# nianticlabs/mickey

Hardware: NVIDIA H100
Metric: image-pairs/sec @720x540 (higher is better)
Workload: dtype f16 operands / f32 accumulate (tensor core), f32 matcher+solver

## Files before the change

### mickey_b200/csrc/epilogue.cuh

```cuda
#pragma once
#include "common.cuh"

namespace mk {

__device__ __forceinline__ float rcp_approx(float x) { float y; asm("rcp.approx.ftz.f32 %0, %1;" : "=f"(y) : "f"(x)); return y; }
__device__ __forceinline__ float ex2_approx_f(float x) { float y; asm("ex2.approx.ftz.f32 %0, %1;" : "=f"(y) : "f"(x)); return y; }
__device__ __forceinline__ float gelu_erf(float x) {
  const float z = fabsf(x) * 0.70710678118654752f;
  const float t = rcp_approx(fmaf(0.3275911f, z, 1.0f));
  float poly = fmaf(1.061405429f, t, -1.453152027f);
  poly = fmaf(poly, t, 1.421413741f);
  poly = fmaf(poly, t, -0.284496736f);
  poly = fmaf(poly, t, 0.254829592f);
  const float erf_abs = fmaf(-poly * t, ex2_approx_f(-1.4426950408889634f * z * z), 1.0f);
  const float hx = 0.5f * x;
  return fmaf(hx, copysignf(erf_abs, x), hx);
}

__device__ __forceinline__ void fma2_f32(float& d0, float& d1, float a0, float a1, float b0, float b1, float c0, float c1) {
  d0 = __fmaf_rn(a0, b0, c0);
  d1 = __fmaf_rn(a1, b1, c1);
}
__device__ __forceinline__ void mul2_f32(float& d0, float& d1, float a0, float a1, float b0, float b1) {
  d0 = __fmul_rn(a0, b0);
// ... 105 lines not shown
        uint4 u = r[q];
        const __half2* h = reinterpret_cast<const __half2*>(&u);
#pragma unroll
        for (int e = 0; e < 4; ++e) {
          float2 f = __half22float2(h[e]);
          v[q * 8 + e * 2] += f.x;
          v[q * 8 + e * 2 + 1] += f.y;
        }
      }
    }
#pragma unroll
    for (int j = 0; j < 32; ++j) v[j] = apply_act(v[j], p.act);
    if (p.aux && ((p.aux_group_mask >> g) & 1)) add_vec32(v, p.aux + (size_t)pos * p.N + n0);
    if (!valid) {
#pragma unroll
      for (int j = 0; j < 32; ++j) v[j] = 0.0f;
    }
    if (p.out_f) {
      float* o = p.out_f + (size_t)g * p.out_f_group_off + (size_t)m * p.out_f_ld + n0;
#pragma unroll
      for (int q = 0; q < 8; ++q)
        reinterpret_cast<float4*>(o)[q] = make_float4(v[q * 4], v[q * 4 + 1], v[q * 4 + 2], v[q * 4 + 3]);
    }
    if (p.out_h) store_h32(p.out_h + (size_t)g * p.out_h_group_off + (size_t)m * p.out_h_ld + n0, v);
  } else if constexpr (EPI == EPI_STORE_F) {
    if (m >= p.M) return;
    float* o = p.out_f + (size_t)g * p.out_f_group_off + (size_t)m * p.out_f_ld + n0;
#pragma unroll
    for (int q = 0; q < 8; ++q)
      reinterpret_cast<float4*>(o)[q] = make_float4(v[q * 4], v[q * 4 + 1], v[q * 4 + 2], v[q * 4 + 3]);
  }
}

template <int CPL> struct VecF;
template <> struct VecF<1> { using T = float; };
template <> struct VecF<2> { using T = float2; };

template <int CPL> __device__ __forceinline__ void ld_f(const float* p, float (&v)[CPL]) {
  if constexpr (CPL == 2) { const float2 t = *reinterpret_cast<const float2*>(p); v[0] = t.x; v[1] = t.y; } else { v[0] = *p; }
}
template <int CPL> __device__ __forceinline__ void ldg_f(const float* p, float (&v)[CPL]) {
  if constexpr (CPL == 2) { const float2 t = __ldg(reinterpret_cast<const float2*>(p)); v[0] = t.x; v[1] = t.y; } else { v[0] = __ldg(p); }
}
template <int CPL> __device__ __forceinline__ void st_f(float* p, const float (&v)[CPL]) {
  if constexpr (CPL == 2) { *reinterpret_cast<float2*>(p) = make_float2(v[0], v[1]); } else { *p = v[0]; }
}
template <int CPL> __device__ __forceinline__ void st_h(__half* p, const float (&v)[CPL]) {
  if constexpr (CPL == 2) { *reinterpret_cast<__half2*>(p) = __floats2half2_rn(v[0], v[1]); } else { *p = __float2half_rn(v[0]); }
}
template <int CPL> __device__ __forceinline__ void ld_h(const __half* p, float (&v)[CPL]) {
  if constexpr (CPL == 2) { const float2 t = __half22float2(*reinterpret_cast<const __half2*>(p)); v[0] = t.x; v[1] = t.y; }
  else { v[0] = __half2float(*p); }
}

__device__ __forceinline__ float warp_rowsum32(float (&part)[32], int lane) {
#pragma unroll
  for (int o = 16; o >= 1; o >>= 1) {
    const bool upper = (lane & o) != 0;
#pragma unroll
    for (int i = 0; i < o; ++i) {
      const float send = upper ? part[i] : part[i + o];
      const float keep = upper ? part[i + o] : part[i];
      part[i] = keep + __shfl_xor_sync(0xffffffffu, send, o);
    }
  }
  return part[0];
}

__device__ __forceinline__ float resid_ln_pass1(const GemmParams& p, int row0, int lane, int col_base, float* stage) {
  constexpr int LDS = 64 + 4, RB = 8;
  const int col = col_base + lane * 2;
  const float2 bias = __ldg(reinterpret_cast<const float2*>(p.bias + col)), gam = __ldg(reinterpret_cast<const float2*>(p.gamma + col));
  const int rows = min(32, p.M - row0);
  float part[32];
#pragma unroll
  for (int r0 = 0; r0 < 32; r0 += RB) {
    float2 v[RB], x[RB];
#pragma unroll
    for (int i = 0; i < RB; ++i) {
      const int r = r0 + i;
      v[i] = *reinterpret_cast<const float2*>(stage + r * LDS + lane * 2);
      x[i] = make_float2(0.f, 0.f);
      if (r < rows) x[i] = *reinterpret_cast<const float2*>(p.out_f + (size_t)(row0 + r) * p.out_f_ld + col);
    }
#pragma unroll
    for (int i = 0; i < RB; ++i) {
      const int r = r0 + i;
      float2 y = make_float2(0.f, 0.f);
      if (r < rows) {
        y.x = fmaf(gam.x, v[i].x + bias.x, x[i].x); y.y = fmaf(gam.y, v[i].y + bias.y, x[i].y);
        *reinterpret_cast<float2*>(p.out_f + (size_t)(row0 + r) * p.out_f_ld + col) = y;
      }
      *reinterpret_cast<float2*>(stage + r * LDS + lane * 2) = y;
      part[r] = y.x + y.y;
    }
  }
  return warp_rowsum32(part, lane);
}

__device__ __forceinline__ float resid_ln_pass2(int lane, const float* stage, float mean_l) {
  constexpr int LDS = 64 + 4;
  float part[32];
#pragma unroll
  for (int r = 0; r < 32; ++r) {
    const float2 x = *reinterpret_cast<const float2*>(stage + r * LDS + lane * 2);
    const float mean = __shfl_sync(0xffffffffu, mean_l, r);
    const float d0 = x.x - mean, d1 = x.y - mean;
    part[r] = d0 * d0 + d1 * d1;
  }
  return warp_rowsum32(part, lane);
}

__device__ __forceinline__ void resid_ln_pass3(const GemmParams& p, int row0, int lane, int col_base, const float* stage,
                                               float mean_l, float rstd_l) {
  constexpr int LDS = 64 + 4;
  const int col = col_base + lane * 2;
  const float2 w = __ldg(reinterpret_cast<const float2*>(p.aux + col)), b = __ldg(reinterpret_cast<const float2*>(p.beta + col));
  const int rows = min(32, p.M - row0);
#pragma unroll 8
  for (int r = 0; r < 32; ++r) {
    const float2 x = *reinterpret_cast<const float2*>(stage + r * LDS + lane * 2);
    const float mean = __shfl_sync(0xffffffffu, mean_l, r), rstd = __shfl_sync(0xffffffffu, rstd_l, r);
    if (r < rows)
      *reinterpret_cast<__half2*>(p.out_h + (size_t)(row0 + r) * p.out_h_ld + col) =
          __floats2half2_rn((x.x - mean) * rstd * w.x + b.x, (x.y - mean) * rstd * w.y + b.y);
  }
}

__device__ __forceinline__ void ld8(const float* p, float (&v)[8]) {
  const float4 a = *reinterpret_cast<const float4*>(p), b = *reinterpret_cast<const float4*>(p + 4);
  v[0] = a.x; v[1] = a.y; v[2] = a.z; v[3] = a.w; v[4] = b.x; v[5] = b.y; v[6] = b.z; v[7] = b.w;
}
__device__ __forceinline__ void ldg8(const float* p, float (&v)[8]) {
  const float4 a = __ldg(reinterpret_cast<const float4*>(p)), b = __ldg(reinterpret_cast<const float4*>(p) + 1);
  v[0] = a.x; v[1] = a.y; v[2] = a.z; v[3] = a.w; v[4] = b.x; v[5] = b.y; v[6] = b.z; v[7] = b.w;
}
__device__ __forceinline__ void st8(float* p, const float (&v)[8]) {
  reinterpret_cast<float4*>(p)[0] = make_float4(v[0], v[1], v[2], v[3]);
  reinterpret_cast<float4*>(p)[1] = make_float4(v[4], v[5], v[6], v[7]);
}
__device__ __forceinline__ void st8h(__half* p, const float (&v)[8]) {
  __half2 h0 = __floats2half2_rn(v[0], v[1]), h1 = __floats2half2_rn(v[2], v[3]);
  __half2 h2 = __floats2half2_rn(v[4], v[5]), h3 = __floats2half2_rn(v[6], v[7]);
  uint4 u;
  u.x = *reinterpret_cast<uint32_t*>(&h0); u.y = *reinterpret_cast<uint32_t*>(&h1);
  u.z = *reinterpret_cast<uint32_t*>(&h2); u.w = *reinterpret_cast<uint32_t*>(&h3);
  *reinterpret_cast<uint4*>(p) = u;
}
__device__ __forceinline__ void ld8h(const __half* p, float (&v)[8]) {
  const uint4 u = *reinterpret_cast<const uint4*>(p);
  const __half2* h = reinterpret_cast<const __half2*>(&u);
#pragma unroll
  for (int e = 0; e < 4; ++e) { const float2 f = __half22float2(h[e]); v[2 * e] = f.x; v[2 * e + 1] = f.y; }
}

template <int EPI, int W, int ACT>
__device__ __forceinline__ void epilogue_rows_impl(const GemmParams& p, int g, int row0, int lane, int col_base,
                                                   const float* __restrict__ stage, float mean_l, float rstd_l) {
  constexpr int LDS = W + 4;
  constexpr int LPR = W / 8;
  constexpr int RPS = 32 / LPR;
  constexpr int STEPS = 32 / RPS;
  constexpr bool GLOBAL_IN = (EPI == EPI_RESID_F || EPI == EPI_PATCH || EPI == EPI_CONV || EPI == EPI_LN);
  constexpr int U = GLOBAL_IN ? 2 : 4;
  static_assert(W % 8 == 0 && 32 % LPR == 0 && STEPS % U == 0, "staged epilogue: W in {32, 64}");
  const int seg = lane % LPR, rsub = lane / LPR;
  const int col = col_base + seg * 8;
  float bias[8], gam[8], bet[8];
#pragma unroll
  for (int i = 0; i < 8; ++i) { bias[i] = 0.f; gam[i] = 1.f; bet[i] = 0.f; }
  if constexpr (EPI == EPI_STORE_H || EPI == EPI_CONV) { if (p.bias) ldg8(p.bias + (size_t)g * p.bias_group_off + col, bias); }
  if constexpr (EPI == EPI_RESID_F) { ldg8(p.bias + col, bias); ldg8(p.gamma + col, gam); }
  if constexpr (EPI == EPI_LN) { ldg8(p.gamma + (size_t)g * p.ln_group_off + col, gam); ldg8(p.beta + (size_t)g * p.ln_group_off + col, bet); }
  const bool use_aux = (EPI == EPI_CONV) && p.aux && ((p.aux_group_mask >> g) & 1);
  const bool use_res = (EPI == EPI_CONV) && p.res_h;
  const bool ln_res = (EPI == EPI_LN) && p.out_f;
  const int rows = min(32, p.M - row0);
  int my_pos = 0, my_valid = 1, my_orow = 0;
  {
    const int mr = row0 + lane;
    if constexpr (EPI == EPI_CONV || EPI == EPI_LN) {
      if (p.pad_h2) { int pos; my_valid = pad_valid(p, mr, pos) ? 1 : 0; my_pos = pos; }
    }
    if constexpr (EPI == EPI_PATCH) {
      const int img = mr / p.tok_per_img;
      my_pos = mr - img * p.tok_per_img;
      my_orow = img * (p.tok_per_img + 1) + 1 + my_pos;
    }
  }
  float* out_f = p.out_f ? p.out_f + (size_t)g * p.out_f_group_off + col : nullptr;
  __half* out_h = p.out_h ? p.out_h + (size_t)g * p.out_h_group_off + col : nullptr;
#pragma unroll 1
  for (int s0 = 0; s0 < STEPS; s0 += U) {
    float v[U][8], x[U][8], a[U][8];
    int pos[U], orow[U];
    bool valid[U], live[U];
    float mean[U], rstd[U];
#pragma unroll
    for (int u = 0; u < U; ++u) {
      const int r = (s0 + u) * RPS + rsub;
      const size_t m = (size_t)(row0 + r);
      live[u] = r < rows;
      ld8(stage + r * LDS + seg * 8, v[u]);
      pos[u] = __shfl_sync(0xffffffffu, my_pos, r);
      orow[u] = __shfl_sync(0xffffffffu, my_orow, r);
      valid[u] = __shfl_sync(0xffffffffu, my_valid, r) != 0;
      mean[u] = 0.f; rstd[u] = 0.f;
      if constexpr (EPI == EPI_LN) { mean[u] = __shfl_sync(0xffffffffu, mean_l, r); rstd[u] = __shfl_sync(0xffffffffu, rstd_l, r); }
#pragma unroll
      for (int k = 0; k < 8; ++k) { x[u][k] = 0.f; a[u][k] = 0.f; }
      if (live[u]) {
        if constexpr (EPI == EPI_RESID_F) ld8(out_f + m * p.out_f_ld, x[u]);
        if constexpr (EPI == EPI_PATCH) ldg8(p.aux + (size_t)pos[u] * p.N + col, a[u]);
        if constexpr (EPI == EPI_CONV) {
          if (use_res) ld8h(p.res_h + (size_t)g * p.res_h_group_off + m * p.res_h_ld + col, x[u]);
          if (use_aux) ldg8(p.aux + (size_t)pos[u] * p.N + col, a[u]);
        }
        if constexpr (EPI == EPI_LN) { if (ln_res) ld8(out_f + m * p.out_f_ld, x[u]); }
      }
    }
#pragma unroll
    for (int u = 0; u < U; ++u) {
      if (!live[u]) continue;
      const int r = (s0 + u) * RPS + rsub;
      const size_t m = (size_t)(row0 + r);
      if constexpr (EPI == EPI_STORE_H) {
        if constexpr (ACT == ACT_GELU) {
#pragma unroll
          for (int k = 0; k < 8; k += 2) gelu_erf2(v[u][k] + bias[k], v[u][k + 1] + bias[k + 1], v[u][k], v[u][k + 1]);
        } else {
#pragma unroll
          for (int k = 0; k < 8; ++k) {
            const float t = v[u][k] + bias[k];
            v[u][k] = (ACT == ACT_RELU) ? fmaxf(t, 0.f) : t;
          }
        }
// ... 216 lines not shown
```

### mickey_b200/csrc/gemm.cu

```cuda
#include "gemm.h"
#include "gemm_tc.cuh"

#include <algorithm>
#include <cstdarg>
#include <cstdlib>
#include <cstring>
#include <mutex>
#include <unordered_map>

namespace mk {

typedef CUresult (*PFN_encodeTiled)(CUtensorMap*, CUtensorMapDataType, cuuint32_t, void*, const cuuint64_t*,
                                    const cuuint64_t*, const cuuint32_t*, const cuuint32_t*, CUtensorMapInterleave,
                                    CUtensorMapSwizzle, CUtensorMapL2promotion, CUtensorMapFloatOOBfill);

static PFN_encodeTiled get_encode() {
  static PFN_encodeTiled fn = nullptr;
  static std::once_flag once;
  std::call_once(once, [] {
    void* p = nullptr;
    cudaDriverEntryPointQueryResult qres;
    if (cudaGetDriverEntryPoint("cuTensorMapEncodeTiled", &p, cudaEnableDefault, &qres) == cudaSuccess &&
        qres == cudaDriverEntryPointSuccess)
      fn = reinterpret_cast<PFN_encodeTiled>(p);
// ... 161 lines not shown
    for (int c = 0; c < BN / 32; ++c) {
      if (n0 + c * 32 < p.N) {
        for (int j = 0; j < 32; ++j) v[j] = acc[c * 32 + j];
        epilogue_chunk<EPI>(p, g, m, n0 + c * 32, v);
      }
    }
  }
}

bool pdl_enabled() {
  static int v = -1;
  if (v < 0) { const char* e = getenv("MICKEY_PDL"); v = (e && strcmp(e, "0") == 0) ? 0 : 1; }
  return v == 1;
}

static bool use_simt() {
  static int v = -1;
  if (v < 0) {
    const char* e = getenv("MICKEY_GEMM_IMPL");
    v = (e && strcmp(e, "simt") == 0) ? 1 : 0;
  }
  return v == 1;
}

int sm_count() {
  static int n[64] = {0};
  int dev = 0;
  cudaGetDevice(&dev);
  int& c = n[dev & 63];
  if (!c) { cudaDeviceGetAttribute(&c, cudaDevAttrMultiProcessorCount, dev); if (c <= 0) c = 132; }
  return c;
}

template <int BN, int EPI, int STAGES, bool PERSISTENT>
static int launch_tc(const CUtensorMap& tmA, const CUtensorMap& tmB, const GemmParams& p, cudaStream_t stream,
                     const OutMaps& om = no_out_maps()) {
  static unsigned long long attr_mask = 0;
  constexpr int smem = gemm_smem_bytes<BN, EPI, STAGES, PERSISTENT>();
  if (first_use_on_device(attr_mask)) {
    MK_CUDA_CHECK(cudaFuncSetAttribute(gemm_tc_kernel<BN, EPI, STAGES, PERSISTENT>, cudaFuncAttributeMaxDynamicSharedMemorySize, smem));
  }
  const int tiles = gemm_tile_count<BN>(p);
  cudaLaunchConfig_t cfg = {};
  cfg.gridDim = dim3(PERSISTENT ? std::min(tiles, sm_count()) : tiles);
  cfg.blockDim = dim3(gemm_threads<PERSISTENT>()); cfg.dynamicSmemBytes = smem; cfg.stream = stream;
  cudaLaunchAttribute attr[2];
  int n_attr = 0;
  if (pdl_enabled()) {
    attr[n_attr].id = cudaLaunchAttributeProgrammaticStreamSerialization;
    attr[n_attr++].val.programmaticStreamSerializationAllowed = 1;
  }
  if constexpr (EPI == EPI_RESID_LN) {
    attr[n_attr].id = cudaLaunchAttributeClusterDimension;
    attr[n_attr].val.clusterDim.x = p.N / BN; attr[n_attr].val.clusterDim.y = 1; attr[n_attr++].val.clusterDim.z = 1;
  }
  cfg.attrs = attr;
  cfg.numAttrs = n_attr;
  MK_CUDA_CHECK(cudaLaunchKernelEx(&cfg, gemm_tc_kernel<BN, EPI, STAGES, PERSISTENT>, tmA, tmB, p, om));
  return MK_OK;
}

static bool deep_ring(int tiles, const GemmParams& p) {
  return (long long)tiles <= (long long)sm_count() * 5 / 4 && p.k_chunks > 3;
}
static bool persistent_grid(int tiles) { return tiles > 8 * sm_count(); }

template <int BN, int EPI>
static int launch_one(const GemmOperand& A, const GemmOperand& B, const GemmParams& p, cudaStream_t stream, int impl) {
  const int tiles = gemm_tile_count<BN>(p);
  if constexpr (EPI == EPI_RESID_LN) {
    if (impl == GEMM_IMPL_SIMT || BN != 128 || p.N / BN > 8 || p.groups != 1) { set_last_error("EPI_RESID_LN: wgmma path, N <= 1024, one group"); return MK_ERR_UNSUPPORTED; }
  }
  if (impl == GEMM_IMPL_SIMT) {
    if constexpr (EPI != EPI_RESID_LN)
    MK_CUDA_CHECK(launch_k(gemm_simt_kernel<BN, EPI>, dim3(tiles), dim3(128), 0, stream, reinterpret_cast<const __half*>(A.ptr),
                           (long long)A.rows, (long long)A.ld, reinterpret_cast<const __half*>(B.ptr), (long long)B.rows,
                           (long long)B.ld, p));
  } else {
    CUtensorMap tmA, tmB;
    int rc = make_tensor_map_f16(&tmA, A.ptr, A.rows, A.cols, A.ld, BLOCK_M);
    if (rc) return rc;
    rc = make_tensor_map_f16(&tmB, B.ptr, B.rows, B.cols, B.ld, BN);
    if (rc) return rc;
    if constexpr (EPI == EPI_DUAL) {
      if (p.out_tma) {
        OutMaps om = {};
        float* outs[3] = {p.scores, p.kp_scores, p.final_scores};
        for (int i = 0; i < 3; ++i)
          if (outs[i]) { rc = encode_tensor_map_out_f32(&om.m[i], outs[i], p.n_valid, p.out_pitch, p.groups); if (rc) return rc; }
        return launch_tc<BN, EPI, shallow_stages<BN>(), false>(tmA, tmB, p, stream, om);
      }
    }
    if (deep_ring(tiles, p)) return launch_tc<BN, EPI, deep_stages<BN>(), false>(tmA, tmB, p, stream);
    if constexpr (persistent_epilogue<EPI>())
      if (persistent_grid(tiles)) return launch_tc<BN, EPI, ring_stages<BN>(), true>(tmA, tmB, p, stream);
    return launch_tc<BN, EPI, shallow_stages<BN>(), false>(tmA, tmB, p, stream);
  }
  MK_CUDA_CHECK(cudaGetLastError());
  return MK_OK;
}

template <int EPI>
static int launch_bn(int bn, const GemmOperand& A, const GemmOperand& B, const GemmParams& p, cudaStream_t s, int impl) {
  if (bn == 128) return launch_one<128, EPI>(A, B, p, s, impl);
  if (bn == 64) return launch_one<64, EPI>(A, B, p, s, impl);
  set_last_error("unsupported BLOCK_N %d", bn);
  return MK_ERR_INVALID;
}

bool gemm_resid_ln_supported(int M, int N, int k_chunks) {
  (void)M; (void)k_chunks;
  static int on = -1;
  if (on < 0) { const char* e = getenv("MICKEY_FUSE_LN"); on = (e && e[0] == '1') ? 1 : 0; }
  return on && !use_simt() && N % 128 == 0 && N <= 1024;
}

int launch_gemm(int epi, const GemmOperand& A, const GemmOperand& B, const GemmParams& p, cudaStream_t stream, int impl) {
  if (impl == GEMM_IMPL_DEFAULT) impl = use_simt() ? GEMM_IMPL_SIMT : GEMM_IMPL_TC;
  if (p.k_chunks <= 0 || p.M <= 0 || p.N <= 0 || p.groups <= 0) { set_last_error("bad GEMM shape"); return MK_ERR_INVALID; }
  const bool matcher = (epi == EPI_LSE || epi == EPI_DUAL);
  if (matcher && impl == GEMM_IMPL_SIMT) { set_last_error("the matcher epilogues run on the wgmma kernel only"); return MK_ERR_UNSUPPORTED; }
  if (matcher && (p.part_ld % 128 || p.part_ld < p.n_valid)) { set_last_error("matcher: part_ld must be n_valid rounded up to 128"); return MK_ERR_INVALID; }
  if (epi == EPI_DUAL && p.out_pitch < p.n_valid) { set_last_error("matcher: out_pitch %lld < n_valid %d", p.out_pitch, p.n_valid); return MK_ERR_INVALID; }
  if (!matcher && (p.N % 32)) { set_last_error("GEMM N=%d must be a multiple of 32", p.N); return MK_ERR_INVALID; }
  int bn = (matcher || p.N % 128 == 0) ? 128 : 64;
  if (!matcher && p.N % bn) { set_last_error("GEMM N=%d not tileable", p.N); return MK_ERR_INVALID; }
  if (epi == EPI_LN && p.N != 128) { set_last_error("EPI_LN needs N == 128"); return MK_ERR_INVALID; }
  if (epi == EPI_RESID_LN && (p.N % 128 || p.N > 1024 || p.groups != 1 || !p.aux || !p.beta || !p.out_h || !p.out_f)) {
// ... 29 lines not shown
```

### mickey_b200/csrc/gemm.h

```cpp
#pragma once
#include "common.cuh"

namespace mk {

struct GemmOperand {
  const void* ptr;
  long long rows, cols, ld;
};

enum GemmImpl : int { GEMM_IMPL_DEFAULT = 0, GEMM_IMPL_TC = 1, GEMM_IMPL_SIMT = 2 };

int make_tensor_map_f16(CUtensorMap* map, const void* ptr, long long rows, long long cols, long long ld_elems, int box_rows);
int encode_tensor_map_2d(CUtensorMap* map, CUtensorMapDataType dtype, const void* ptr, long long rows, long long cols,
                         long long ld_elems, int box_rows);
int make_tensor_map_out_f16(CUtensorMap* map, void* ptr, long long groups, long long rows, long long cols, int box_rows);
int sm_count();
int launch_gemm(int epi, const GemmOperand& A, const GemmOperand& B, const GemmParams& p, cudaStream_t stream,
                int impl = GEMM_IMPL_DEFAULT);
bool gemm_resid_ln_supported(int M, int N, int k_chunks);
const char* last_error();

}
```

### mickey_b200/csrc/gemm_tc.cuh

```cuda
#pragma once
#include "common.cuh"
#include "epilogue.cuh"

namespace mk {

constexpr int BLOCK_M = 128;
constexpr int BLOCK_K = 64;
constexpr int WGMMA_K = 16;
constexpr int GEMM_WARP_EPI = 8;

template <int BN> constexpr int ring_stages() { return BN == 128 ? 4 : 6; }
template <int BN> constexpr int shallow_stages() { return BN == 128 ? 3 : 4; }
template <int BN> constexpr int deep_stages() { return BN == 128 ? 6 : 8; }
template <int EPI> constexpr bool persistent_epilogue() { return EPI != EPI_DUAL && EPI != EPI_RESID_LN && EPI != EPI_LN; }
template <bool PERSISTENT> constexpr int gemm_threads() { return PERSISTENT ? 640 : 288; }
template <bool PERSISTENT> constexpr int gemm_warp_tma() { return PERSISTENT ? 16 : 8; }

constexpr int DUAL_STAGE_BYTES = 3 * 4096;
constexpr int DUAL_AUX_BYTES = 8 * 64 * 4;
constexpr int DUAL_BYTES = 8 * DUAL_STAGE_BYTES + DUAL_AUX_BYTES;

template <int BN> constexpr int acc_block_floats() { return 32 * (BN / 2 + 4); }
template <int BN> constexpr int acc_tile_bytes() { return 8 * acc_block_floats<BN>() * 4; }
template <int BN, int STAGES> constexpr int ring_bytes() { return STAGES * (BLOCK_M * BLOCK_K * 2 + BN * BLOCK_K * 2); }
template <int BN, int EPI, int STAGES, bool PERSISTENT> constexpr int acc_tile_offset() {
  return PERSISTENT ? ring_bytes<BN, STAGES>() : EPI == EPI_DUAL ? DUAL_BYTES : 0;
}
template <int BN, int EPI, int STAGES, bool PERSISTENT>
constexpr int region_bytes() {
  return ring_bytes<BN, STAGES>() > acc_tile_offset<BN, EPI, STAGES, PERSISTENT>() + acc_tile_bytes<BN>()
             ? ring_bytes<BN, STAGES>() : acc_tile_offset<BN, EPI, STAGES, PERSISTENT>() + acc_tile_bytes<BN>();
}
template <int BN, int EPI, int STAGES, bool PERSISTENT> constexpr int gemm_smem_bytes() {
  return region_bytes<BN, EPI, STAGES, PERSISTENT>() + 1024 + 256 + 2048;
}
template <int BN, int EPI, int STAGES, bool PERSISTENT> constexpr int gemm_ctas_per_sm() {
  return !PERSISTENT && EPI != EPI_LN && EPI != EPI_RESID_LN && gemm_smem_bytes<BN, EPI, STAGES, PERSISTENT>() <= 113 * 1024 ? 2 : 1;
}

struct GemmTile { int g, m0, n0, n_tile; };
template <int BN>
__host__ __device__ __forceinline__ int gemm_tile_count(const GemmParams& p) {
  return ((p.M + BLOCK_M - 1) / BLOCK_M) * ((p.N + BN - 1) / BN) * p.groups;
}
template <int BN>
__device__ __forceinline__ GemmTile gemm_tile(const GemmParams& p, int t) {
  const int n_tiles = (p.N + BN - 1) / BN, m_tiles = (p.M + BLOCK_M - 1) / BLOCK_M;
  const int n = t % n_tiles;
  t /= n_tiles;
  int g, m;
  if (p.a_row_group_off == 0 && p.a_col_group_off == 0) { g = t % p.groups; m = t / p.groups; }
  else { m = t % m_tiles; g = t / m_tiles; }
  return {g, m * BLOCK_M, n * BN, n};
}

__device__ __forceinline__ uint32_t smem_u32(const void* p) { return (uint32_t)__cvta_generic_to_shared(p); }

__device__ __forceinline__ void mbar_init(uint32_t bar, uint32_t count) {
  asm volatile("mbarrier.init.shared::cta.b64 [%0], %1;" ::"r"(bar), "r"(count));
}
__device__ __forceinline__ void mbar_expect_tx(uint32_t bar, uint32_t bytes) {
  asm volatile("mbarrier.arrive.expect_tx.shared::cta.b64 _, [%0], %1;" ::"r"(bar), "r"(bytes) : "memory");
}
__device__ __forceinline__ void mbar_arrive(uint32_t bar) {
  asm volatile("mbarrier.arrive.shared::cta.b64 _, [%0];" ::"r"(bar) : "memory");
}
__device__ __forceinline__ void mbar_wait(uint32_t bar, uint32_t parity) {
  asm volatile(
      "{\n\t"
      ".reg .pred P1;\n\t"
      "WAIT_%=:\n\t"
      "mbarrier.try_wait.parity.shared::cta.b64 P1, [%0], %1;\n\t"
      "@P1 bra DONE_%=;\n\t"
      "bra WAIT_%=;\n\t"
      "DONE_%=:\n\t"
      "}" ::"r"(bar), "r"(parity) : "memory");
}
__device__ __forceinline__ void tma_load_2d(uint32_t dst, const CUtensorMap* map, uint32_t bar, int c0, int c1) {
  asm volatile(
      "cp.async.bulk.tensor.2d.shared::cluster.global.mbarrier::complete_tx::bytes [%0], [%1, {%3, %4}], [%2];"
      ::"r"(dst), "l"(map), "r"(bar), "r"(c0), "r"(c1) : "memory");
}
__device__ __forceinline__ bool elect_one() {
  uint32_t pred = 0;
  asm volatile(
      "{\n\t"
      ".reg .pred P1;\n\t"
      "elect.sync _|P1, 0xFFFFFFFF;\n\t"
      "selp.b32 %0, 1, 0, P1;\n\t"
      "}" : "=r"(pred));
  return pred != 0;
}
constexpr int GEMM_REGS_PRODUCER = 40;
constexpr int GEMM_REGS_EPILOGUE = 120;
template <int R> __device__ __forceinline__ void setmaxnreg_dec() { asm volatile("setmaxnreg.dec.sync.aligned.u32 %0;" ::"n"(R)); }
template <int R> __device__ __forceinline__ void setmaxnreg_inc() { asm volatile("setmaxnreg.inc.sync.aligned.u32 %0;" ::"n"(R)); }
__device__ __forceinline__ void consumer_sync() { asm volatile("bar.sync 1, 256;" ::: "memory"); }

__device__ __forceinline__ uint64_t gmma_desc_sw128(uint32_t smem_addr) {
  uint64_t d = 0;
  d |= (uint64_t)((smem_addr & 0x3FFFF) >> 4);
  d |= (uint64_t)1 << 16;
  d |= (uint64_t)(1024 >> 4) << 32;
  d |= (uint64_t)1 << 62;
  return d;
}
__device__ __forceinline__ void wgmma_fence() { asm volatile("wgmma.fence.sync.aligned;" ::: "memory"); }
__device__ __forceinline__ void wgmma_commit() { asm volatile("wgmma.commit_group.sync.aligned;" ::: "memory"); }
template <int N> __device__ __forceinline__ void wgmma_wait() { asm volatile("wgmma.wait_group.sync.aligned %0;" ::"n"(N) : "memory"); }
template <int N> __device__ __forceinline__ void reg_fence(float (&d)[N]) {
#pragma unroll
  for (int i = 0; i < N; ++i) asm volatile("" : "+f"(d[i])::"memory");
}

__device__ __forceinline__ void wgmma_m64n64k16(float (&d)[32], uint64_t desc_a, uint64_t desc_b, uint32_t scale_d) {
// ... 9 lines not shown
  asm volatile(
      "{\n\t.reg .pred p;\n\tsetp.ne.b32 p, %66, 0;\n\t"
      "wgmma.mma_async.sync.aligned.m64n128k16.f32.f16.f16 "
      "{%0, %1, %2, %3, %4, %5, %6, %7, %8, %9, %10, %11, %12, %13, %14, %15, %16, %17, %18, %19, %20, %21, %22, %23, %24, %25, %26, %27, %28, %29, %30, %31, %32, %33, %34, %35, %36, %37, %38, %39, %40, %41, %42, %43, %44, %45, %46, %47, %48, %49, %50, %51, %52, %53, %54, %55, %56, %57, %58, %59, %60, %61, %62, %63}, %64, %65, p, 1, 1, 0, 0;\n\t}"
      : "+f"(d[0]), "+f"(d[1]), "+f"(d[2]), "+f"(d[3]), "+f"(d[4]), "+f"(d[5]), "+f"(d[6]), "+f"(d[7]), "+f"(d[8]), "+f"(d[9]), "+f"(d[10]), "+f"(d[11]), "+f"(d[12]), "+f"(d[13]), "+f"(d[14]), "+f"(d[15]), "+f"(d[16]), "+f"(d[17]), "+f"(d[18]), "+f"(d[19]), "+f"(d[20]), "+f"(d[21]), "+f"(d[22]), "+f"(d[23]), "+f"(d[24]), "+f"(d[25]), "+f"(d[26]), "+f"(d[27]), "+f"(d[28]), "+f"(d[29]), "+f"(d[30]), "+f"(d[31]), "+f"(d[32]), "+f"(d[33]), "+f"(d[34]), "+f"(d[35]), "+f"(d[36]), "+f"(d[37]), "+f"(d[38]), "+f"(d[39]), "+f"(d[40]), "+f"(d[41]), "+f"(d[42]), "+f"(d[43]), "+f"(d[44]), "+f"(d[45]), "+f"(d[46]), "+f"(d[47]), "+f"(d[48]), "+f"(d[49]), "+f"(d[50]), "+f"(d[51]), "+f"(d[52]), "+f"(d[53]), "+f"(d[54]), "+f"(d[55]), "+f"(d[56]), "+f"(d[57]), "+f"(d[58]), "+f"(d[59]), "+f"(d[60]), "+f"(d[61]), "+f"(d[62]), "+f"(d[63])
      : "l"(desc_a), "l"(desc_b), "r"(scale_d));
}

template <int BN>
__device__ __forceinline__ void wgmma_tile(float (&d)[BN / 2], uint64_t desc_a, uint64_t desc_b, uint32_t scale_d) {
  if constexpr (BN == 128) wgmma_m64n128k16(d, desc_a, desc_b, scale_d);
  else wgmma_m64n64k16(d, desc_a, desc_b, scale_d);
}

__device__ __forceinline__ void cluster_sync_all() {
  asm volatile("barrier.cluster.arrive.release.aligned;\n\tbarrier.cluster.wait.acquire.aligned;" ::: "memory");
}
__device__ __forceinline__ uint32_t cluster_size() {
  uint32_t r;
  asm volatile("mov.u32 %0, %%cluster_nctarank;" : "=r"(r));
  return r;
}
__device__ __forceinline__ float ld_dsmem_f32(uint32_t local_smem_addr, uint32_t cta_rank) {
  uint32_t remote;
  asm volatile("mapa.shared::cluster.u32 %0, %1, %2;" : "=r"(remote) : "r"(local_smem_addr), "r"(cta_rank));
  float v;
  asm volatile("ld.shared::cluster.f32 %0, [%1];" : "=f"(v) : "r"(remote) : "memory");
  return v;
}

template <int BN>
__device__ __forceinline__ void acc_chunk(const float* acc, int q, int lane, int c, float (&v)[32]) {
  constexpr int W = BN / 2;
  const float4* src = reinterpret_cast<const float4*>(acc + (q + 4 * ((c * 32) / W)) * acc_block_floats<BN>() + lane * (W + 4) + (c * 32) % W);
#pragma unroll
  for (int k4 = 0; k4 < 8; ++k4) {
    const float4 t = src[k4];
    v[k4 * 4] = t.x; v[k4 * 4 + 1] = t.y; v[k4 * 4 + 2] = t.z; v[k4 * 4 + 3] = t.w;
  }
}

template <int BN, int EPI>
__device__ __forceinline__ void tile_epilogue(const GemmParams& p, const OutMaps& om, int g, int m0, int n0, int n_tile, int q, int half,
                                              int lane, float* acc, float* red, uint32_t red_saddr, float* dual_stage, float* dual_aux) {
  constexpr int CHUNKS = BN / 32;
  constexpr int W = BN / 2;
  constexpr int CPH = CHUNKS / 2;
  const int c_begin = half * CPH, c_end = c_begin + CPH;
  const int m = m0 + q * 32 + lane;
  float* stage = acc + (q + 4 * half) * acc_block_floats<BN>();
  float v[32];
  if constexpr (EPI == EPI_LN) {
    float sum = 0.f;
#pragma unroll
    for (int c = 0; c < CHUNKS; ++c) {
      acc_chunk<BN>(acc, q, lane, c, v);
#pragma unroll
      for (int j = 0; j < 32; ++j) sum += v[j];
    }
    const float mean = sum * (1.0f / BN);
    float sq = 0.f;
#pragma unroll
    for (int c = 0; c < CHUNKS; ++c) {
      acc_chunk<BN>(acc, q, lane, c, v);
#pragma unroll
      for (int j = 0; j < 32; ++j) { const float d = v[j] - mean; sq += d * d; }
    }
    const float rstd = rsqrtf(sq * (1.0f / BN) + p.eps);
    epilogue_rows<EPI_LN, W>(p, g, m0 + q * 32, lane, n0 + half * W, stage, mean, rstd);
  } else if constexpr (EPI == EPI_RESID_LN) {
// ... 41 lines not shown
    const bool row_ok = m < p.n_valid;
    const float lr = row_ok ? __ldg(p.lse_r + (size_t)g * p.part_ld + m) : -MK_NEG_INF;
    const float s0 = row_ok ? __ldg(p.scr0 + (size_t)g * p.n_valid + m) : 0.0f;
    if (p.out_tma) {
      float lc_pre[CPH], s1_pre[CPH];
#pragma unroll
      for (int ci = 0; ci < CPH; ++ci) {
        const int col = n0 + (c_begin + ci) * 32 + lane;
        const bool ok = col < p.n_valid;
        lc_pre[ci] = ok ? __ldg(p.lse_c + (size_t)g * p.part_ld + col) : -MK_NEG_INF;
        s1_pre[ci] = ok ? __ldg(p.scr1 + (size_t)g * p.n_valid + col) : 0.0f;
      }
#pragma unroll
      for (int ci = 0; ci < CPH; ++ci) {
        const int c = c_begin + ci;
        if (n0 + c * 32 < p.n_valid && m0 + q * 32 < p.n_valid) {
          acc_chunk<BN>(acc, q, lane, c, v);
          dual_store_chunk_tma(p, om, g, m0 + q * 32, lane, n0 + c * 32, v, dual_stage, dual_aux, lr, s0, lc_pre[ci], s1_pre[ci]);
        }
      }
    } else {
      for (int c = c_begin; c < c_end; ++c) {
        if (n0 + c * 32 < p.n_valid) {
          acc_chunk<BN>(acc, q, lane, c, v);
          dual_store_chunk(p, g, m0 + q * 32, lane, n0 + c * 32, v, dual_stage, lr, s0);
        }
      }
    }
  } else {
    epilogue_rows<EPI, W>(p, g, m0 + q * 32, lane, n0 + half * W, stage, 0.f, 0.f);
  }
}

template <int BN, int EPI, int STAGES, bool PERSISTENT>
__global__ void __launch_bounds__((gemm_threads<PERSISTENT>()), (gemm_ctas_per_sm<BN, EPI, STAGES, PERSISTENT>()))
gemm_tc_kernel(const __grid_constant__ CUtensorMap tmA, const __grid_constant__ CUtensorMap tmB, const GemmParams p,
               const __grid_constant__ OutMaps om) {
  static_assert(BN == 64 || BN == 128, "wgmma tiles: N = 64 or 128");
  static_assert(gemm_smem_bytes<BN, EPI, STAGES, PERSISTENT>() <= 227 * 1024, "GEMM: shared memory");
  extern __shared__ uint8_t smem_raw[];
  constexpr int A_BYTES = BLOCK_M * BLOCK_K * 2;
  constexpr int B_BYTES = BN * BLOCK_K * 2;
  constexpr int STAGE_BYTES = A_BYTES + B_BYTES;
  constexpr int W = BN / 2;
  static_assert(!PERSISTENT || persistent_epilogue<EPI>(), "this epilogue runs one tile per CTA");
  constexpr bool ONE_TILE = !PERSISTENT;
  constexpr int WARP_TMA = gemm_warp_tma<PERSISTENT>();

  const uint32_t raw = smem_u32(smem_raw);
  const uint32_t base = (raw + 1023u) & ~1023u;
  const uint32_t bar_base = base + region_bytes<BN, EPI, STAGES, PERSISTENT>();
  const uint32_t full_bar0 = bar_base;
  const uint32_t empty_bar0 = bar_base + 8 * STAGES;
  const uint32_t acc_full_bar = bar_base + 16 * STAGES;
  const uint32_t acc_empty_bar = acc_full_bar + 8;
  const uint32_t red_saddr = bar_base + 256;
  uint8_t* const gbase = smem_raw + (base - raw);
  float* const acc = reinterpret_cast<float*>(gbase + acc_tile_offset<BN, EPI, STAGES, PERSISTENT>());

  const int warp = threadIdx.x >> 5;
  const int lane = threadIdx.x & 31;
  const int n_tiles_total = gemm_tile_count<BN>(p);

  if (warp == WARP_TMA && lane == 0) {
    asm volatile("prefetch.tensormap [%0];" ::"l"(&tmA) : "memory");
    asm volatile("prefetch.tensormap [%0];" ::"l"(&tmB) : "memory");
    for (int s = 0; s < STAGES; ++s) {
      mbar_init(full_bar0 + 8 * s, 1);
      mbar_init(empty_bar0 + 8 * s, 8);
    }
    mbar_init(acc_full_bar, 256);
    mbar_init(acc_empty_bar, 256);
    asm volatile("fence.mbarrier_init.release.cluster;" ::: "memory");
  }
  __syncthreads();
  pdl_wait();

  if (warp >= WARP_TMA) {
    if constexpr (!ONE_TILE) setmaxnreg_dec<GEMM_REGS_PRODUCER>();
    if (warp == WARP_TMA && elect_one()) {
      int stage = 0;
      uint32_t phase = 0;
      for (int t = blockIdx.x; t < n_tiles_total; t += gridDim.x) {
        const GemmTile tile = gemm_tile<BN>(p, t);
        const int a_col0 = p.a_col_base + tile.g * p.a_col_group_off;
        const int a_row0 = tile.m0 + tile.g * p.a_row_group_off;
        const int b_row0 = tile.n0 + tile.g * p.b_row_group_off;
        for (int kc = 0; kc < p.k_chunks; ++kc) {
          const int tap = kc / p.chunks_per_tap;
          const int kin = kc - tap * p.chunks_per_tap;
          mbar_wait(empty_bar0 + 8 * stage, phase ^ 1);
          const uint32_t sa = base + stage * STAGE_BYTES;
          const uint32_t fb = full_bar0 + 8 * stage;
          mbar_expect_tx(fb, STAGE_BYTES);
          tma_load_2d(sa, &tmA, fb, a_col0 + kin * BLOCK_K, a_row0 + p.tap_shift[tap]);
          tma_load_2d(sa + A_BYTES, &tmB, fb, kc * BLOCK_K, b_row0);
          if (++stage == STAGES) { stage = 0; phase ^= 1; }
        }
      }
    }
    __syncwarp();
    pdl_trigger();
    if constexpr (EPI == EPI_RESID_LN) { cluster_sync_all(); cluster_sync_all(); cluster_sync_all(); }
    return;
  }

  if (warp < GEMM_WARP_EPI) {
    const int wg = warp >> 2;
    int stage = 0;
    uint32_t phase = 0, acc_phase = 0;
    for (int t = blockIdx.x; t < n_tiles_total; t += gridDim.x) {
      float d[BN / 2];
#pragma unroll
      for (int i = 0; i < BN / 2; ++i) d[i] = 0.f;
      for (int kc = 0; kc < p.k_chunks; ++kc) {
        mbar_wait(full_bar0 + 8 * stage, phase);
        const uint32_t sa = base + stage * STAGE_BYTES;
        const uint64_t da = gmma_desc_sw128(sa + wg * (64 * 128));
        const uint64_t db = gmma_desc_sw128(sa + A_BYTES);
        wgmma_fence();
#pragma unroll
        for (int k = 0; k < BLOCK_K / WGMMA_K; ++k)
          wgmma_tile<BN>(d, da + (uint64_t)(k * 2), db + (uint64_t)(k * 2), 1u);
        wgmma_commit();
        wgmma_wait<1>();
        reg_fence(d);
        if (kc > 0 && lane == 0) mbar_arrive(empty_bar0 + 8 * (stage == 0 ? STAGES - 1 : stage - 1));
        if (++stage == STAGES) { stage = 0; phase ^= 1; }
      }
      wgmma_wait<0>();
      reg_fence(d);
      if (lane == 0) mbar_arrive(empty_bar0 + 8 * (stage == 0 ? STAGES - 1 : stage - 1));
      if (t + (int)gridDim.x >= n_tiles_total) pdl_trigger();

      if constexpr (ONE_TILE) consumer_sync();
      else mbar_wait(acc_empty_bar, acc_phase ^ 1);
      const int r_base = wg * 64 + (warp & 3) * 16 + (lane >> 2);
#pragma unroll
      for (int j = 0; j < BN / 8; ++j) {
#pragma unroll
        for (int h = 0; h < 2; ++h) {
          const int r = r_base + 8 * h, c = 8 * j + 2 * (lane & 3);
          float* dst = acc + ((r >> 5) + 4 * (c / W)) * acc_block_floats<BN>() + (r & 31) * (W + 4) + (c % W);
          *reinterpret_cast<float2*>(dst) = make_float2(d[4 * j + 2 * h], d[4 * j + 2 * h + 1]);
        }
      }
      if constexpr (ONE_TILE) {
        consumer_sync();
        const GemmTile tile = gemm_tile<BN>(p, t);
        tile_epilogue<BN, EPI>(p, om, tile.g, tile.m0, tile.n0, tile.n_tile, warp & 3, warp >> 2, lane, acc,
                               reinterpret_cast<float*>(smem_raw + (red_saddr - raw)), red_saddr,
                               reinterpret_cast<float*>(gbase + warp * DUAL_STAGE_BYTES),
                               reinterpret_cast<float*>(gbase + 8 * DUAL_STAGE_BYTES) + warp * 64);
      } else {
        mbar_arrive(acc_full_bar);
        acc_phase ^= 1;
      }
    }
    if constexpr (EPI == EPI_DUAL) { if (p.out_tma && lane == 0) tma_store_wait_all(); }
    return;
  }

  if constexpr (ONE_TILE) return;
  setmaxnreg_inc<GEMM_REGS_EPILOGUE>();
  const int ew = warp - GEMM_WARP_EPI;
  uint32_t acc_phase = 0;
  for (int t = blockIdx.x; t < n_tiles_total; t += gridDim.x) {
    const GemmTile tile = gemm_tile<BN>(p, t);
    mbar_wait(acc_full_bar, acc_phase);
    if (t + (int)gridDim.x >= n_tiles_total) pdl_trigger();
    tile_epilogue<BN, EPI>(p, om, tile.g, tile.m0, tile.n0, tile.n_tile, ew & 3, ew >> 2, lane, acc,
                           reinterpret_cast<float*>(smem_raw + (red_saddr - raw)), red_saddr,
                           reinterpret_cast<float*>(gbase + ew * DUAL_STAGE_BYTES),
                           reinterpret_cast<float*>(gbase + 8 * DUAL_STAGE_BYTES) + ew * 64);
    mbar_arrive(acc_empty_bar);
    acc_phase ^= 1;
  }
}

}
```

Baseline: 296.6.

## Pair CTAs in clusters to multicast B tiles and swizzle accumulator staging

Adds a two-CTA cluster mode for the persistent GEMM. Each CTA loads half of the shared B tile and multicasts it to both CTAs, and consumers release ring slots on both CTAs' empty barriers, which cuts global/L2 traffic for B. The persistent path is now chosen ahead of the deep-ring path and is paired by default. Separately, the padded accumulator staging layout (row stride W+4) is replaced by an XOR swizzle (acc_idx), which drops the padding while aiming to avoid shared-memory bank conflicts. Risks are cross-CTA barrier coupling, M-tail CTAs doing idle work, and the reordered dispatch.

```diff
diff --git a/mickey_b200/csrc/epilogue.cuh b/mickey_b200/csrc/epilogue.cuh
--- a/mickey_b200/csrc/epilogue.cuh
+++ b/mickey_b200/csrc/epilogue.cuh
@@ -161,6 +161,12 @@
   }
 }
 
+template <int W> __device__ __forceinline__ int acc_idx(int r, int c) {
+  const int k = c >> 2;
+  const int h = 2 * (r & 3) + ((r ^ (r >> 2) ^ (k >> 3)) & 1);
+  return r * W + ((k ^ h) << 2) + (c & 3);
+}
+
 template <int CPL> struct VecF;
 template <> struct VecF<1> { using T = float; };
 template <> struct VecF<2> { using T = float2; };
@@ -197,7 +203,7 @@
 }
 
 __device__ __forceinline__ float resid_ln_pass1(const GemmParams& p, int row0, int lane, int col_base, float* stage) {
-  constexpr int LDS = 64 + 4, RB = 8;
+  constexpr int RB = 8;
   const int col = col_base + lane * 2;
   const float2 bias = __ldg(reinterpret_cast<const float2*>(p.bias + col)), gam = __ldg(reinterpret_cast<const float2*>(p.gamma + col));
   const int rows = min(32, p.M - row0);
@@ -208,7 +214,7 @@
 #pragma unroll
     for (int i = 0; i < RB; ++i) {
       const int r = r0 + i;
-      v[i] = *reinterpret_cast<const float2*>(stage + r * LDS + lane * 2);
+      v[i] = *reinterpret_cast<const float2*>(stage + acc_idx<64>(r, lane * 2));
       x[i] = make_float2(0.f, 0.f);
       if (r < rows) x[i] = *reinterpret_cast<const float2*>(p.out_f + (size_t)(row0 + r) * p.out_f_ld + col);
     }
@@ -220,7 +226,7 @@
         y.x = fmaf(gam.x, v[i].x + bias.x, x[i].x); y.y = fmaf(gam.y, v[i].y + bias.y, x[i].y);
         *reinterpret_cast<float2*>(p.out_f + (size_t)(row0 + r) * p.out_f_ld + col) = y;
       }
-      *reinterpret_cast<float2*>(stage + r * LDS + lane * 2) = y;
+      *reinterpret_cast<float2*>(stage + acc_idx<64>(r, lane * 2)) = y;
       part[r] = y.x + y.y;
     }
   }
@@ -228,11 +234,10 @@
 }
 
 __device__ __forceinline__ float resid_ln_pass2(int lane, const float* stage, float mean_l) {
-  constexpr int LDS = 64 + 4;
   float part[32];
 #pragma unroll
   for (int r = 0; r < 32; ++r) {
-    const float2 x = *reinterpret_cast<const float2*>(stage + r * LDS + lane * 2);
+    const float2 x = *reinterpret_cast<const float2*>(stage + acc_idx<64>(r, lane * 2));
     const float mean = __shfl_sync(0xffffffffu, mean_l, r);
     const float d0 = x.x - mean, d1 = x.y - mean;
     part[r] = d0 * d0 + d1 * d1;
@@ -242,13 +247,12 @@
 
 __device__ __forceinline__ void resid_ln_pass3(const GemmParams& p, int row0, int lane, int col_base, const float* stage,
                                                float mean_l, float rstd_l) {
-  constexpr int LDS = 64 + 4;
   const int col = col_base + lane * 2;
   const float2 w = __ldg(reinterpret_cast<const float2*>(p.aux + col)), b = __ldg(reinterpret_cast<const float2*>(p.beta + col));
   const int rows = min(32, p.M - row0);
 #pragma unroll 8
   for (int r = 0; r < 32; ++r) {
-    const float2 x = *reinterpret_cast<const float2*>(stage + r * LDS + lane * 2);
+    const float2 x = *reinterpret_cast<const float2*>(stage + acc_idx<64>(r, lane * 2));
     const float mean = __shfl_sync(0xffffffffu, mean_l, r), rstd = __shfl_sync(0xffffffffu, rstd_l, r);
     if (r < rows)
       *reinterpret_cast<__half2*>(p.out_h + (size_t)(row0 + r) * p.out_h_ld + col) =
@@ -286,7 +290,6 @@
 template <int EPI, int W, int ACT>
 __device__ __forceinline__ void epilogue_rows_impl(const GemmParams& p, int g, int row0, int lane, int col_base,
                                                    const float* __restrict__ stage, float mean_l, float rstd_l) {
-  constexpr int LDS = W + 4;
   constexpr int LPR = W / 8;
   constexpr int RPS = 32 / LPR;
   constexpr int STEPS = 32 / RPS;
@@ -330,7 +333,11 @@
       const int r = (s0 + u) * RPS + rsub;
       const size_t m = (size_t)(row0 + r);
       live[u] = r < rows;
-      ld8(stage + r * LDS + seg * 8, v[u]);
+      {
+        const float4 a = *reinterpret_cast<const float4*>(stage + acc_idx<W>(r, seg * 8));
+        const float4 b = *reinterpret_cast<const float4*>(stage + acc_idx<W>(r, seg * 8 + 4));
+        v[u][0] = a.x; v[u][1] = a.y; v[u][2] = a.z; v[u][3] = a.w; v[u][4] = b.x; v[u][5] = b.y; v[u][6] = b.z; v[u][7] = b.w;
+      }
       pos[u] = __shfl_sync(0xffffffffu, my_pos, r);
       orow[u] = __shfl_sync(0xffffffffu, my_orow, r);
       valid[u] = __shfl_sync(0xffffffffu, my_valid, r) != 0;
diff --git a/mickey_b200/csrc/gemm.cu b/mickey_b200/csrc/gemm.cu
--- a/mickey_b200/csrc/gemm.cu
+++ b/mickey_b200/csrc/gemm.cu
@@ -217,31 +217,46 @@
   return c;
 }
 
-template <int BN, int EPI, int STAGES, bool PERSISTENT>
+template <int BN, int EPI, int STAGES, bool PERSISTENT, bool PAIR = false>
 static int launch_tc(const CUtensorMap& tmA, const CUtensorMap& tmB, const GemmParams& p, cudaStream_t stream,
                      const OutMaps& om = no_out_maps()) {
   static unsigned long long attr_mask = 0;
+  static int max_clusters[64] = {0};
   constexpr int smem = gemm_smem_bytes<BN, EPI, STAGES, PERSISTENT>();
-  if (first_use_on_device(attr_mask)) {
-    MK_CUDA_CHECK(cudaFuncSetAttribute(gemm_tc_kernel<BN, EPI, STAGES, PERSISTENT>, cudaFuncAttributeMaxDynamicSharedMemorySize, smem));
-  }
-  const int tiles = gemm_tile_count<BN>(p);
+  auto kernel = gemm_tc_kernel<BN, EPI, STAGES, PERSISTENT, PAIR>;
   cudaLaunchConfig_t cfg = {};
-  cfg.gridDim = dim3(PERSISTENT ? std::min(tiles, sm_count()) : tiles);
   cfg.blockDim = dim3(gemm_threads<PERSISTENT>()); cfg.dynamicSmemBytes = smem; cfg.stream = stream;
   cudaLaunchAttribute attr[2];
   int n_attr = 0;
+  if constexpr (EPI == EPI_RESID_LN || PAIR) {
+    attr[n_attr].id = cudaLaunchAttributeClusterDimension;
+    attr[n_attr].val.clusterDim.x = PAIR ? 2 : p.N / BN; attr[n_attr].val.clusterDim.y = 1; attr[n_attr++].val.clusterDim.z = 1;
+  }
+  cfg.attrs = attr;
+  cfg.numAttrs = n_attr;
+  int dev = 0;
+  if constexpr (PAIR) cudaGetDevice(&dev);
+  if (first_use_on_device(attr_mask)) {
+    MK_CUDA_CHECK(cudaFuncSetAttribute(kernel, cudaFuncAttributeMaxDynamicSharedMemorySize, smem));
+    if constexpr (PAIR) {
+      cfg.gridDim = dim3(2 * sm_count());
+      MK_CUDA_CHECK(cudaOccupancyMaxActiveClusters(&max_clusters[dev & 63], kernel, &cfg));
+    }
+  }
+  const int tiles = gemm_tile_count<BN>(p);
+  if constexpr (PAIR) {
+    const int n_clusters = max_clusters[dev & 63];
+    if (n_clusters <= 0) { set_last_error("GEMM: no two-CTA cluster of %d bytes of shared memory fits on this device", smem); return MK_ERR_UNSUPPORTED; }
+    cfg.gridDim = dim3(2 * std::min(gemm_tile_count<BN, 2>(p), n_clusters));
+  } else {
+    cfg.gridDim = dim3(PERSISTENT ? std::min(tiles, sm_count()) : tiles);
+  }
   if (pdl_enabled()) {
     attr[n_attr].id = cudaLaunchAttributeProgrammaticStreamSerialization;
     attr[n_attr++].val.programmaticStreamSerializationAllowed = 1;
   }
-  if constexpr (EPI == EPI_RESID_LN) {
-    attr[n_attr].id = cudaLaunchAttributeClusterDimension;
-    attr[n_attr].val.clusterDim.x = p.N / BN; attr[n_attr].val.clusterDim.y = 1; attr[n_attr++].val.clusterDim.z = 1;
-  }
-  cfg.attrs = attr;
   cfg.numAttrs = n_attr;
-  MK_CUDA_CHECK(cudaLaunchKernelEx(&cfg, gemm_tc_kernel<BN, EPI, STAGES, PERSISTENT>, tmA, tmB, p, om));
+  MK_CUDA_CHECK(cudaLaunchKernelEx(&cfg, kernel, tmA, tmB, p, om));
   return MK_OK;
 }
 
@@ -265,6 +280,16 @@
     CUtensorMap tmA, tmB;
     int rc = make_tensor_map_f16(&tmA, A.ptr, A.rows, A.cols, A.ld, BLOCK_M);
     if (rc) return rc;
+    if constexpr (persistent_epilogue<EPI>()) {
+      const bool forced = impl == GEMM_IMPL_TC_PAIRED || impl == GEMM_IMPL_TC_UNPAIRED;
+      if (forced || persistent_grid(tiles)) {
+        const bool pair = impl != GEMM_IMPL_TC_UNPAIRED;
+        rc = make_tensor_map_f16(&tmB, B.ptr, B.rows, B.cols, B.ld, pair ? BN / 2 : BN);
+        if (rc) return rc;
+        if (pair) return launch_tc<BN, EPI, ring_stages<BN>(), true, true>(tmA, tmB, p, stream);
+        return launch_tc<BN, EPI, ring_stages<BN>(), true>(tmA, tmB, p, stream);
+      }
+    }
     rc = make_tensor_map_f16(&tmB, B.ptr, B.rows, B.cols, B.ld, BN);
     if (rc) return rc;
     if constexpr (EPI == EPI_DUAL) {
@@ -277,8 +302,6 @@
       }
     }
     if (deep_ring(tiles, p)) return launch_tc<BN, EPI, deep_stages<BN>(), false>(tmA, tmB, p, stream);
-    if constexpr (persistent_epilogue<EPI>())
-      if (persistent_grid(tiles)) return launch_tc<BN, EPI, ring_stages<BN>(), true>(tmA, tmB, p, stream);
     return launch_tc<BN, EPI, shallow_stages<BN>(), false>(tmA, tmB, p, stream);
   }
   MK_CUDA_CHECK(cudaGetLastError());
diff --git a/mickey_b200/csrc/gemm.h b/mickey_b200/csrc/gemm.h
--- a/mickey_b200/csrc/gemm.h
+++ b/mickey_b200/csrc/gemm.h
@@ -8,7 +8,7 @@
   long long rows, cols, ld;
 };
 
-enum GemmImpl : int { GEMM_IMPL_DEFAULT = 0, GEMM_IMPL_TC = 1, GEMM_IMPL_SIMT = 2 };
+enum GemmImpl : int { GEMM_IMPL_DEFAULT = 0, GEMM_IMPL_TC = 1, GEMM_IMPL_SIMT = 2, GEMM_IMPL_TC_PAIRED = 3, GEMM_IMPL_TC_UNPAIRED = 4 };
 
 int make_tensor_map_f16(CUtensorMap* map, const void* ptr, long long rows, long long cols, long long ld_elems, int box_rows);
 int encode_tensor_map_2d(CUtensorMap* map, CUtensorMapDataType dtype, const void* ptr, long long rows, long long cols,
diff --git a/mickey_b200/csrc/gemm_tc.cuh b/mickey_b200/csrc/gemm_tc.cuh
--- a/mickey_b200/csrc/gemm_tc.cuh
+++ b/mickey_b200/csrc/gemm_tc.cuh
@@ -20,7 +20,7 @@
 constexpr int DUAL_AUX_BYTES = 8 * 64 * 4;
 constexpr int DUAL_BYTES = 8 * DUAL_STAGE_BYTES + DUAL_AUX_BYTES;
 
-template <int BN> constexpr int acc_block_floats() { return 32 * (BN / 2 + 4); }
+template <int BN> constexpr int acc_block_floats() { return 32 * (BN / 2); }
 template <int BN> constexpr int acc_tile_bytes() { return 8 * acc_block_floats<BN>() * 4; }
 template <int BN, int STAGES> constexpr int ring_bytes() { return STAGES * (BLOCK_M * BLOCK_K * 2 + BN * BLOCK_K * 2); }
 template <int BN, int EPI, int STAGES, bool PERSISTENT> constexpr int acc_tile_offset() {
@@ -39,19 +39,19 @@
 }
 
 struct GemmTile { int g, m0, n0, n_tile; };
-template <int BN>
+template <int BN, int MT = 1>
 __host__ __device__ __forceinline__ int gemm_tile_count(const GemmParams& p) {
-  return ((p.M + BLOCK_M - 1) / BLOCK_M) * ((p.N + BN - 1) / BN) * p.groups;
-}
-template <int BN>
-__device__ __forceinline__ GemmTile gemm_tile(const GemmParams& p, int t) {
-  const int n_tiles = (p.N + BN - 1) / BN, m_tiles = (p.M + BLOCK_M - 1) / BLOCK_M;
+  return ((p.M + MT * BLOCK_M - 1) / (MT * BLOCK_M)) * ((p.N + BN - 1) / BN) * p.groups;
+}
+template <int BN, int MT = 1>
+__device__ __forceinline__ GemmTile gemm_tile(const GemmParams& p, int t, int rank = 0) {
+  const int n_tiles = (p.N + BN - 1) / BN, m_units = (p.M + MT * BLOCK_M - 1) / (MT * BLOCK_M);
   const int n = t % n_tiles;
   t /= n_tiles;
   int g, m;
   if (p.a_row_group_off == 0 && p.a_col_group_off == 0) { g = t % p.groups; m = t / p.groups; }
-  else { m = t % m_tiles; g = t / m_tiles; }
-  return {g, m * BLOCK_M, n * BN, n};
+  else { m = t % m_units; g = t / m_units; }
+  return {g, (m * MT + rank) * BLOCK_M, n * BN, n};
 }
 
 __device__ __forceinline__ uint32_t smem_u32(const void* p) { return (uint32_t)__cvta_generic_to_shared(p); }
@@ -81,6 +81,19 @@
       "cp.async.bulk.tensor.2d.shared::cluster.global.mbarrier::complete_tx::bytes [%0], [%1, {%3, %4}], [%2];"
       ::"r"(dst), "l"(map), "r"(bar), "r"(c0), "r"(c1) : "memory");
 }
+__device__ __forceinline__ void tma_load_2d_multicast(uint32_t dst, const CUtensorMap* map, uint32_t bar, int c0, int c1,
+                                                      uint16_t cta_mask) {
+  asm volatile(
+      "cp.async.bulk.tensor.2d.shared::cluster.global.mbarrier::complete_tx::bytes.multicast::cluster [%0], [%1, {%3, %4}], [%2], %5;"
+      ::"r"(dst), "l"(map), "r"(bar), "r"(c0), "r"(c1), "h"(cta_mask) : "memory");
+}
+__device__ __forceinline__ void mbar_arrive_cluster(uint32_t bar, uint32_t cta_rank) {
+  asm volatile(
+      "{\n\t.reg .b32 remote;\n\t"
+      "mapa.shared::cluster.u32 remote, %0, %1;\n\t"
+      "mbarrier.arrive.shared::cluster.b64 _, [remote];\n\t}"
+      ::"r"(bar), "r"(cta_rank) : "memory");
+}
 __device__ __forceinline__ bool elect_one() {
   uint32_t pred = 0;
   asm volatile(
@@ -156,10 +169,10 @@
 template <int BN>
 __device__ __forceinline__ void acc_chunk(const float* acc, int q, int lane, int c, float (&v)[32]) {
   constexpr int W = BN / 2;
-  const float4* src = reinterpret_cast<const float4*>(acc + (q + 4 * ((c * 32) / W)) * acc_block_floats<BN>() + lane * (W + 4) + (c * 32) % W);
+  const float* blk = acc + (q + 4 * ((c * 32) / W)) * acc_block_floats<BN>();
 #pragma unroll
   for (int k4 = 0; k4 < 8; ++k4) {
-    const float4 t = src[k4];
+    const float4 t = *reinterpret_cast<const float4*>(blk + acc_idx<W>(lane, (c * 32) % W + 4 * k4));
     v[k4 * 4] = t.x; v[k4 * 4 + 1] = t.y; v[k4 * 4 + 2] = t.z; v[k4 * 4 + 3] = t.w;
   }
 }
@@ -267,7 +280,7 @@
   }
 }
 
-template <int BN, int EPI, int STAGES, bool PERSISTENT>
+template <int BN, int EPI, int STAGES, bool PERSISTENT, bool PAIR = false>
 __global__ void __launch_bounds__((gemm_threads<PERSISTENT>()), (gemm_ctas_per_sm<BN, EPI, STAGES, PERSISTENT>()))
 gemm_tc_kernel(const __grid_constant__ CUtensorMap tmA, const __grid_constant__ CUtensorMap tmB, const GemmParams p,
                const __grid_constant__ OutMaps om) {
@@ -279,8 +292,13 @@
   constexpr int STAGE_BYTES = A_BYTES + B_BYTES;
   constexpr int W = BN / 2;
   static_assert(!PERSISTENT || persistent_epilogue<EPI>(), "this epilogue runs one tile per CTA");
+  static_assert(!PAIR || PERSISTENT, "CTA pairs: persistent kernel only");
   constexpr bool ONE_TILE = !PERSISTENT;
   constexpr int WARP_TMA = gemm_warp_tma<PERSISTENT>();
+  constexpr int MT = PAIR ? 2 : 1;
+  const int rank = PAIR ? (int)(blockIdx.x & 1) : 0;
+  const int work0 = PAIR ? (int)(blockIdx.x >> 1) : (int)blockIdx.x;
+  const int work_step = PAIR ? (int)(gridDim.x >> 1) : (int)gridDim.x;
 
   const uint32_t raw = smem_u32(smem_raw);
   const uint32_t base = (raw + 1023u) & ~1023u;
@@ -295,20 +313,21 @@
 
   const int warp = threadIdx.x >> 5;
   const int lane = threadIdx.x & 31;
-  const int n_tiles_total = gemm_tile_count<BN>(p);
+  const int n_work = gemm_tile_count<BN, MT>(p);
 
   if (warp == WARP_TMA && lane == 0) {
     asm volatile("prefetch.tensormap [%0];" ::"l"(&tmA) : "memory");
     asm volatile("prefetch.tensormap [%0];" ::"l"(&tmB) : "memory");
     for (int s = 0; s < STAGES; ++s) {
       mbar_init(full_bar0 + 8 * s, 1);
-      mbar_init(empty_bar0 + 8 * s, 8);
+      mbar_init(empty_bar0 + 8 * s, 8 * MT);
     }
     mbar_init(acc_full_bar, 256);
     mbar_init(acc_empty_bar, 256);
     asm volatile("fence.mbarrier_init.release.cluster;" ::: "memory");
   }
-  __syncthreads();
+  if constexpr (PAIR) cluster_sync_all();
+  else __syncthreads();
   pdl_wait();
 
   if (warp >= WARP_TMA) {
@@ -316,8 +335,8 @@
     if (warp == WARP_TMA && elect_one()) {
       int stage = 0;
       uint32_t phase = 0;
-      for (int t = blockIdx.x; t < n_tiles_total; t += gridDim.x) {
-        const GemmTile tile = gemm_tile<BN>(p, t);
+      for (int t = work0; t < n_work; t += work_step) {
+        const GemmTile tile = gemm_tile<BN, MT>(p, t, rank);
         const int a_col0 = p.a_col_base + tile.g * p.a_col_group_off;
         const int a_row0 = tile.m0 + tile.g * p.a_row_group_off;
         const int b_row0 = tile.n0 + tile.g * p.b_row_group_off;
@@ -329,7 +348,8 @@
           const uint32_t fb = full_bar0 + 8 * stage;
           mbar_expect_tx(fb, STAGE_BYTES);
           tma_load_2d(sa, &tmA, fb, a_col0 + kin * BLOCK_K, a_row0 + p.tap_shift[tap]);
-          tma_load_2d(sa + A_BYTES, &tmB, fb, kc * BLOCK_K, b_row0);
+          if constexpr (PAIR) tma_load_2d_multicast(sa + A_BYTES + rank * (B_BYTES / 2), &tmB, fb, kc * BLOCK_K, b_row0 + rank * (BN / 2), 0x3);
+          else tma_load_2d(sa + A_BYTES, &tmB, fb, kc * BLOCK_K, b_row0);
           if (++stage == STAGES) { stage = 0; phase ^= 1; }
         }
       }
@@ -337,6 +357,7 @@
     __syncwarp();
     pdl_trigger();
     if constexpr (EPI == EPI_RESID_LN) { cluster_sync_all(); cluster_sync_all(); cluster_sync_all(); }
+    if constexpr (PAIR) cluster_sync_all();
     return;
   }
 
@@ -344,7 +365,11 @@
     const int wg = warp >> 2;
     int stage = 0;
     uint32_t phase = 0, acc_phase = 0;
-    for (int t = blockIdx.x; t < n_tiles_total; t += gridDim.x) {
+    auto release = [&](int s) {
+      if constexpr (PAIR) { mbar_arrive_cluster(empty_bar0 + 8 * s, 0); mbar_arrive_cluster(empty_bar0 + 8 * s, 1); }
+      else mbar_arrive(empty_bar0 + 8 * s);
+    };
+    for (int t = work0; t < n_work; t += work_step) {
       float d[BN / 2];
 #pragma unroll
       for (int i = 0; i < BN / 2; ++i) d[i] = 0.f;
@@ -360,13 +385,13 @@
         wgmma_commit();
         wgmma_wait<1>();
         reg_fence(d);
-        if (kc > 0 && lane == 0) mbar_arrive(empty_bar0 + 8 * (stage == 0 ? STAGES - 1 : stage - 1));
+        if (kc > 0 && lane == 0) release(stage == 0 ? STAGES - 1 : stage - 1);
         if (++stage == STAGES) { stage = 0; phase ^= 1; }
       }
       wgmma_wait<0>();
       reg_fence(d);
-      if (lane == 0) mbar_arrive(empty_bar0 + 8 * (stage == 0 ? STAGES - 1 : stage - 1));
-      if (t + (int)gridDim.x >= n_tiles_total) pdl_trigger();
+      if (lane == 0) release(stage == 0 ? STAGES - 1 : stage - 1);
+      if (t + work_step >= n_work) pdl_trigger();
 
       if constexpr (ONE_TILE) consumer_sync();
       else mbar_wait(acc_empty_bar, acc_phase ^ 1);
@@ -376,7 +401,7 @@
 #pragma unroll
         for (int h = 0; h < 2; ++h) {
           const int r = r_base + 8 * h, c = 8 * j + 2 * (lane & 3);
-          float* dst = acc + ((r >> 5) + 4 * (c / W)) * acc_block_floats<BN>() + (r & 31) * (W + 4) + (c % W);
+          float* dst = acc + ((r >> 5) + 4 * (c / W)) * acc_block_floats<BN>() + acc_idx<W>(r & 31, c % W);
           *reinterpret_cast<float2*>(dst) = make_float2(d[4 * j + 2 * h], d[4 * j + 2 * h + 1]);
         }
       }
@@ -393,6 +418,7 @@
       }
     }
     if constexpr (EPI == EPI_DUAL) { if (p.out_tma && lane == 0) tma_store_wait_all(); }
+    if constexpr (PAIR) cluster_sync_all();
     return;
   }
 
@@ -400,17 +426,19 @@
   setmaxnreg_inc<GEMM_REGS_EPILOGUE>();
   const int ew = warp - GEMM_WARP_EPI;
   uint32_t acc_phase = 0;
-  for (int t = blockIdx.x; t < n_tiles_total; t += gridDim.x) {
-    const GemmTile tile = gemm_tile<BN>(p, t);
+  for (int t = work0; t < n_work; t += work_step) {
+    const GemmTile tile = gemm_tile<BN, MT>(p, t, rank);
     mbar_wait(acc_full_bar, acc_phase);
-    if (t + (int)gridDim.x >= n_tiles_total) pdl_trigger();
-    tile_epilogue<BN, EPI>(p, om, tile.g, tile.m0, tile.n0, tile.n_tile, ew & 3, ew >> 2, lane, acc,
-                           reinterpret_cast<float*>(smem_raw + (red_saddr - raw)), red_saddr,
-                           reinterpret_cast<float*>(gbase + ew * DUAL_STAGE_BYTES),
-                           reinterpret_cast<float*>(gbase + 8 * DUAL_STAGE_BYTES) + ew * 64);
+    if (t + work_step >= n_work) pdl_trigger();
+    if (tile.m0 < p.M)
+      tile_epilogue<BN, EPI>(p, om, tile.g, tile.m0, tile.n0, tile.n_tile, ew & 3, ew >> 2, lane, acc,
+                             reinterpret_cast<float*>(smem_raw + (red_saddr - raw)), red_saddr,
+                             reinterpret_cast<float*>(gbase + ew * DUAL_STAGE_BYTES),
+                             reinterpret_cast<float*>(gbase + 8 * DUAL_STAGE_BYTES) + ew * 64);
     mbar_arrive(acc_empty_bar);
     acc_phase ^= 1;
   }
-}
-
-}
+  if constexpr (PAIR) cluster_sync_all();
+}
+
+}
```

New measurement: 307.4 (median of 6 runs). 1.04x the previous value.
